# loop-Z/omniisaacgymenvs_loop

Measured on AMD Instinct MI355X. Metric: env-steps/sec USV_CaptureXY at 1/2/4/8 MI355X; wall-clock to reward=30, higher is better.
Workload: dtype fp32; 1 GPU; USV_Virtual_CaptureXY num_envs=131072/GPU PPO-MLP fp32 (BASELINE configs[4] per GPU: 2^20 envs over 8 GPUs); num_envs_per_gpu=131072, horizon_length=16, minibatch_size=8192, mini_epochs=8, parallelism=dp1, exchange=none (one rank), seed=0, full=False

## Files before the change

### omniisaacgymenvs_loop_amd/csrc/usv_field.hip

```cpp
#include "usv_device.h"

USV_PROBE_DEFINE(field)

namespace {

constexpr int G = USV_GRID;
constexpr int G2 = USV_GRID2;
constexpr int FS = USV_FIELD_STRIDE;
constexpr int T = 10;
constexpr int NT = G / T;
constexpr int kWaveThreads = 256;
constexpr int kMaxIters = 4096;
constexpr int kSlotStride = USV_FIELD_SLOT_STATS;
constexpr int kSlotObst = 160;
static_assert(kSlotObst + 2 * USV_NOBST <= kSlotStride, "slot_stats layout");
constexpr int kFieldPackMinEnvs = 32768;
#ifndef USV_SWEEP_WAVES
#define USV_SWEEP_WAVES 2
#endif
constexpr int kPackGrid = 256 * USV_SWEEP_WAVES;

enum {
  SS_GMIN_F = 0, SS_GMAX_F, SS_ANY_INF,
  SS_JMIN_F_NI, SS_JMAX_F_NI, SS_JMAX_F_ALL,
  SS_JRMIN_I_NI, SS_JRMAX_I_NI, SS_JRMAX_I_ALL,
  SS_INSIDE, SS_ITERS, SS_EXACT
};

__device__ __forceinline__ float wall(const uint32_t *freem, int bit) {
  const uint32_t f = (freem[bit >> 5] >> (bit & 31)) & 1u;
  return __uint_as_float((f - 1u) & 0x7f800000u);
}

constexpr int NTP = NT + 2;
constexpr uint32_t kInfBits = 0x7f800000u;
constexpr uint32_t kOcc = 0xFFFFFFFFu;
enum { E_TOP = 0, E_BOT, E_LEFT, E_RIGHT };
constexpr int kOccColWords = (G + 31) / 32;
__device__ __forceinline__ bool occ_bit(const uint32_t *occ, int r, int cc) {
  return (occ[cc * kOccColWords + (r >> 5)] >> (r & 31)) & 1u;
}

constexpr int kRefSweeps = (G * 3) / 2;
template <int NT>
__device__ __forceinline__ void cost_sweeps_exact(const uint32_t *occ, int ix, int iy, float *A, float *B) {
  const int tid = threadIdx.x;
  for (int q = tid; q < G2; q += NT) A[q] = (q == iy * G + ix) ? 0.f : INFINITY;
  __syncthreads();
  for (int it = 0; it < kRefSweeps; ++it) {
    for (int q = tid; q < G2; q += NT) {
      const int r = q / G, cc = q % G;
      float m = A[q];
#pragma unroll
      for (int dy = -1; dy <= 1; ++dy)
#pragma unroll
        for (int dx = -1; dx <= 1; ++dx) {
          if (!dx && !dy) continue;
          const int rr = r - dy, c2 = cc - dx;
          if (rr < 0 || rr >= G || c2 < 0 || c2 >= G) continue;
          m = fminf(m, A[rr * G + c2] + ((dx && dy) ? 1.414f : 1.0f));
        }
      const bool o = r == 0 || r == G - 1 || cc == 0 || cc == G - 1 || occ_bit(occ, r, cc);
      B[q] = o ? INFINITY : m;
    }
    __syncthreads();
    float *t = A; A = B; B = t;
  }
}

constexpr int kPlaceTB = 256;
__global__ __launch_bounds__(kPlaceTB) void k_field_place(usv_cfg_t c, usv_bufs_t b) {
  if (b.ctl[USV_CTL_PLACE] == 0) return;
  const int n = b.n;
  const int count = min(b.ctl[USV_CTL_RESET_COUNT], n);
  const uint64_t h_seed = (uint64_t)(uint32_t)b.ctl[USV_CTL_H_SEED_LO] | ((uint64_t)(uint32_t)b.ctl[USV_CTL_H_SEED_HI] << 32);
  const uint64_t h_step = (uint64_t)(uint32_t)b.ctl[USV_CTL_H_STEP_LO] | ((uint64_t)(uint32_t)b.ctl[USV_CTL_H_STEP_HI] << 32);
  const float *h_inj = reinterpret_cast<const float *>(
      (uintptr_t)((uint64_t)(uint32_t)b.ctl[USV_CTL_H_INJ_LO] | ((uint64_t)(uint32_t)b.ctl[USV_CTL_H_INJ_HI] << 32)));
  const int lane = threadIdx.x & 63;
  const int waves = (int)gridDim.x * (kPlaceTB / 64);
  for (int slot = (int)blockIdx.x * (kPlaceTB / 64) + (int)(threadIdx.x >> 6); slot < count; slot += waves) {
    const int e = b.reset_ids[slot];
    const float2 oc = place_obstacles(c, e, b.px[e], b.py[e], b.field_old_tgt[e], b.field_old_tgt[n + e], h_seed,
                                      h_step, h_inj);
    if (lane < USV_NOBST) {
      b.obst[(size_t)(2 * lane) * n + e] = oc.x;
      b.obst[(size_t)(2 * lane + 1) * n + e] = oc.y;
    }
  }
}

#define USV_SWEEP_NOTE(hb, m) (chg = __builtin_amdgcn_bitop3_b32(chg, (uint32_t)(hb), (uint32_t)(m), 0xF6))
template <bool kPlace, int TH = T, int TW = T, int NTHR = kWaveThreads>
__device__ __forceinline__ void field_wave_body(const usv_cfg_t &c, const usv_bufs_t &b) {
  constexpr int NTR = G / TH, NTC = G / TW;
  constexpr int NPR = NTR + 2, NPC = NTC + 2;
  constexpr int WC = NTHR / 128;
  static_assert(G % TH == 0 && G % TW == 0 && NTR <= 16 && NTC <= 8 * WC && NTHR % 128 == 0, "sweep tiling");
  static_assert(USV_FIELD_TH == TH && USV_FIELD_TW % TW == 0, "sweep tiles inside the field tiles");
  __shared__ uint32_t occ[G * kOccColWords];
  __shared__ float edgeh[2][NPR * NPC][TW];
  __shared__ float edgev[2][NPR * NPC][TH];
  __shared__ int lastc[NPR * NPC];
  __shared__ float so[2 * USV_NOBST];
  __shared__ float slin[G];
  const int n = b.n;
  const int count = min(b.ctl[USV_CTL_RESET_COUNT], n);
  const int tid = threadIdx.x;
  const int lane = tid & 63, wid = tid >> 6;
  const bool place = kPlace && b.ctl[USV_CTL_PLACE] != 0;
  uint64_t h_seed = 0, h_step = 0;
  const float *h_inj = nullptr;
  if (kPlace) {
    h_seed = (uint64_t)(uint32_t)b.ctl[USV_CTL_H_SEED_LO] | ((uint64_t)(uint32_t)b.ctl[USV_CTL_H_SEED_HI] << 32);
    h_step = (uint64_t)(uint32_t)b.ctl[USV_CTL_H_STEP_LO] | ((uint64_t)(uint32_t)b.ctl[USV_CTL_H_STEP_HI] << 32);
    h_inj = reinterpret_cast<const float *>(
        (uintptr_t)((uint64_t)(uint32_t)b.ctl[USV_CTL_H_INJ_LO] | ((uint64_t)(uint32_t)b.ctl[USV_CTL_H_INJ_HI] << 32)));
  }
  const int quad = tid >> 6, qk = tid & 63;
  const int qr = quad / WC, qc = quad % WC;
  const int qw = min(8, NTC - 8 * qc), qh = min(8, NTR - 8 * qr);
  const bool tile_ok = qk < qw * qh;
  const int tr = tile_ok ? qr * 8 + qk / qw : 0;
  const int tc = tile_ok ? qc * 8 + qk % qw : 0;
  const int r0 = tr * TH, c0 = tc * TW;
  const int tp = (tr + 1) * NPC + tc + 1;
  const float cell = (float)((double)c.map_size / G);
  const float half_map = (float)((double)c.map_size / 2);
  const float inv_r = (float)(1.0 / (double)c.influence_radius);
  for (int q = tid; q < 2 * NPR * NPC * TW; q += NTHR) {
    const int t = (q / TW) % (NPR * NPC);
    const int rr = t / NPC, cc = t % NPC;
    if (rr == 0 || rr == NPR - 1 || cc == 0 || cc == NPC - 1) (&edgeh[0][0][0])[q] = INFINITY;
  }
  for (int q = tid; q < 2 * NPR * NPC * TH; q += NTHR) {
    const int t = (q / TH) % (NPR * NPC);
    const int rr = t / NPC, cc = t % NPC;
    if (rr == 0 || rr == NPR - 1 || cc == 0 || cc == NPC - 1) (&edgev[0][0][0])[q] = INFINITY;
  }
  for (int q = tid; q < NPR * NPC; q += NTHR) lastc[q] = -1000;
  for (int slot = blockIdx.x; slot < count; slot += gridDim.x) {
    USV_PHASE(field, 0);
    const int e = b.reset_ids[slot];
    if (kPlace && place) {
      if (wid == 0) {
        const float2 oc = place_obstacles(c, e, b.px[e], b.py[e], b.field_old_tgt[e], b.field_old_tgt[n + e],
                                          h_seed, h_step, h_inj);
        if (lane < USV_NOBST) {
          so[2 * lane] = oc.x;
          so[2 * lane + 1] = oc.y;
          b.obst[(size_t)(2 * lane) * n + e] = oc.x;
          b.obst[(size_t)(2 * lane + 1) * n + e] = oc.y;
        }
      }
    } else if (tid < 2 * USV_NOBST) {
      so[tid] = b.obst[(size_t)tid * n + e];
    }
    if (tid < G) slin[tid] = grid_coord(b.grid_lin, c.map_size, tid);
    for (int q = tid; q < G * kOccColWords; q += NTHR) occ[q] = 0u;
    __syncthreads();
#ifdef USV_PHASE_PROBE
    if (tid == 0 && blockIdx.x < 4096) g_probe_field[blockIdx.x][12] = wall_clock64();
#endif
    if (tid < 2 * USV_NOBST) b.slot_stats[(size_t)slot * kSlotStride + kSlotObst + tid] = so[tid];
    {
      const float half_m = (float)((double)c.map_size / 2);
      const float cellf = (float)((double)c.map_size / G);
      const int reach = (int)ceilf(c.obstacle_radius / cellf) + 2;
      const int bw = 2 * reach + 1;
      for (int q = tid; q < USV_NOBST * bw * bw; q += NTHR) {
        const int o = q / (bw * bw), k = q % (bw * bw);
        const float ox = so[2 * o], oy = so[2 * o + 1];
        const float ic = (ox + half_m) / cellf - 0.5f, jc = (oy + half_m) / cellf - 0.5f;
        if (!(fabsf(ic) < 4.0f * G && fabsf(jc) < 4.0f * G)) continue;
        const int cc = (int)floorf(ic) - reach + k % bw, r = (int)floorf(jc) - reach + k / bw;
        if (cc < 0 || cc >= G || r < 0 || r >= G) continue;
        const float dx = slin[cc] - ox, dy = slin[r] - oy;
        if (sqrtf(fmaf(dy, dy, dx * dx)) - c.obstacle_radius <= 0.f)
          atomicOr(&occ[cc * kOccColWords + (r >> 5)], 1u << (r & 31));
      }
    }
    __syncthreads();
    USV_PHASE(field, 1);
#ifdef USV_PHASE_PROBE
    if (tid == 0 && blockIdx.x < 4096) g_probe_field[blockIdx.x][13] = clock64();
#endif
    const float tx = b.field_old_tgt[e], ty = b.field_old_tgt[n + e];
    int ix = (int)((tx + half_map) / cell), iy = (int)((ty + half_map) / cell);
    ix = min(max(ix, 0), G - 1);
    iy = min(max(iy, 0), G - 1);
    const bool tgt_free = !occ_bit(occ, iy, ix) && ix > 0 && ix < G - 1 && iy > 0 && iy < G - 1;
    float h[TH + 2][TW + 2];
    if (tile_ok) {
#pragma unroll
      for (int i = 0; i < TH; ++i)
#pragma unroll
        for (int j = 0; j < TW; ++j) {
          const int r = r0 + i, cc = c0 + j;
          const bool border = r == 0 || r == G - 1 || cc == 0 || cc == G - 1;
          const bool o = border || occ_bit(occ, r, cc);
          float init = INFINITY;
          if (o) {
            init = __uint_as_float(kOcc);
          } else if (tgt_free) {
            if (r == iy && cc == ix) init = 0.f;
          } else {
            const int di = r - iy, dj = cc - ix;
            if (abs(di) <= 1 && abs(dj) <= 1 && (di || dj)) init = (di && dj) ? 1.414f : 1.0f;
          }
          h[i + 1][j + 1] = init;
        }
#pragma unroll
      for (int k = 0; k < TW; ++k) {
        edgeh[E_TOP][tp][k] = h[1][k + 1];
        edgeh[E_BOT][tp][k] = h[TH][k + 1];
      }
#pragma unroll
      for (int k = 0; k < TH; ++k) {
        edgev[E_LEFT - 2][tp][k] = h[k + 1][1];
        edgev[E_RIGHT - 2][tp][k] = h[k + 1][TW];
      }
      lastc[tp] = 0;
    }
    __syncthreads();
    int it = 0;
    for (; it < kMaxIters; ++it) {
      int changed = 0;
      uint32_t chg = 0u;
      bool dirty = false;
      if (tile_ok) {
#pragma unroll
        for (int dr = -1; dr <= 1; ++dr)
#pragma unroll
          for (int dc = -1; dc <= 1; ++dc) dirty |= lastc[tp + dr * NPC + dc] >= it - 1;
      }
      if (dirty) {
#pragma unroll
        for (int k = 0; k < TW; ++k) {
          h[0][k + 1] = edgeh[E_BOT][tp - NPC][k];
          h[TH + 1][k + 1] = edgeh[E_TOP][tp + NPC][k];
        }
#pragma unroll
        for (int k = 0; k < TH; ++k) {
          h[k + 1][0] = edgev[E_RIGHT - 2][tp - 1][k];
          h[k + 1][TW + 1] = edgev[E_LEFT - 2][tp + 1][k];
        }
        h[0][0] = edgeh[E_BOT][tp - NPC - 1][TW - 1];
        h[0][TW + 1] = edgeh[E_BOT][tp - NPC + 1][0];
        h[TH + 1][0] = edgeh[E_TOP][tp + NPC - 1][TW - 1];
        h[TH + 1][TW + 1] = edgeh[E_TOP][tp + NPC + 1][0];
#pragma unroll
        for (int L = 0; L < 2 * TH + TW - 2; ++L)
#pragma unroll
          for (int i = 1; i <= TH; ++i) {
            const int j = L - 2 * (i - 1) + 1;
            if (j < 1 || j > TW) continue;
            const int32_t hb = __float_as_int(h[i][j]);
            int32_t m = min(hb, __float_as_int(fabsf(h[i - 1][j - 1]) + 1.414f));
            m = min(m, __float_as_int(fabsf(h[i - 1][j]) + 1.0f));
            m = min(m, __float_as_int(fabsf(h[i - 1][j + 1]) + 1.414f));
            m = min(m, __float_as_int(fabsf(h[i][j - 1]) + 1.0f));
            if (i == 1 || i == TH || j == 1 || j == TW) USV_SWEEP_NOTE(hb, m);
            h[i][j] = __int_as_float(m);
          }
#pragma unroll
        for (int L = 0; L < 2 * TH + TW - 2; ++L)
#pragma unroll
          for (int i = TH; i >= 1; --i) {
            const int j = TW - (L - 2 * (TH - i));
            if (j < 1 || j > TW) continue;
            const int32_t hb = __float_as_int(h[i][j]);
            int32_t m = min(hb, __float_as_int(fabsf(h[i + 1][j + 1]) + 1.414f));
            m = min(m, __float_as_int(fabsf(h[i + 1][j]) + 1.0f));
            m = min(m, __float_as_int(fabsf(h[i + 1][j - 1]) + 1.414f));
            m = min(m, __float_as_int(fabsf(h[i][j + 1]) + 1.0f));
            USV_SWEEP_NOTE(hb, m);
            h[i][j] = __int_as_float(m);
          }
        __asm__("" : "+v"(chg));
        changed = chg != 0u;
        if (changed) {
#pragma unroll
          for (int k = 0; k < TW; ++k) {
            edgeh[E_TOP][tp][k] = h[1][k + 1];
            edgeh[E_BOT][tp][k] = h[TH][k + 1];
          }
#pragma unroll
          for (int k = 0; k < TH; ++k) {
            edgev[E_LEFT - 2][tp][k] = h[k + 1][1];
            edgev[E_RIGHT - 2][tp][k] = h[k + 1][TW];
          }
          lastc[tp] = it;
        }
      }
      if (!__syncthreads_or(changed)) break;
    }
    USV_PHASE(field, 2);
#ifdef USV_PHASE_PROBE
    if (tid == 0 && blockIdx.x < 4096) g_probe_field[blockIdx.x][14] = clock64();
#endif
    constexpr float kPinnedCost = 224.0f;
    float hmax = 0.f;
    if (tile_ok) {
#pragma unroll
      for (int i = 0; i < TH; ++i)
#pragma unroll
        for (int j = 0; j < TW; ++j) {
          const uint32_t hb = __float_as_uint(h[i + 1][j + 1]);
          if (hb < kInfBits) hmax = fmaxf(hmax, h[i + 1][j + 1]);
        }
    }
    const bool exact = __syncthreads_or((hmax > kPinnedCost) || (it >= kMaxIters)) != 0;
    constexpr int kSub = USV_FIELD_TW / TW;
    static_assert(USV_FIELD_TCOLS * USV_FIELD_TW == G && USV_FIELD_TCOLS == NTC / kSub, "field tiles = sweep tiles");
    if (tile_ok) {
      float *Ft = b.field + (size_t)e * FS + (tr * USV_FIELD_TCOLS + tc / kSub) * (USV_FIELD_TH * USV_FIELD_TW) +
                  (tc % kSub) * TW;
#pragma unroll
      for (int i = 0; i < TH; ++i)
#pragma unroll
        for (int j = 0; j < TW; ++j)
          Ft[i * USV_FIELD_TW + j] = __float_as_uint(h[i + 1][j + 1]) > kInfBits ? INFINITY : h[i + 1][j + 1];
    }
    if (tile_ok) lastc[tp] = -1000;
    if (exact) {
      __syncthreads();
      float *Fe = b.field + (size_t)e * FS;
      float *scratch = b.sdf + (size_t)e * FS;
      cost_sweeps_exact<NTHR>(occ, ix, iy, Fe, scratch);
      for (int q = tid; q < G2; q += NTHR) Fe[field_idx(q / G, q % G)] = scratch[q];
      if (tid == 0) atomicAdd(&b.ctl[USV_CTL_FIELD_EXACT], 1);
    }
    if (tid == 0) {
      b.slot_stats[(size_t)slot * kSlotStride + SS_ITERS] = (float)it;
      b.slot_stats[(size_t)slot * kSlotStride + SS_EXACT] = exact ? 1.f : 0.f;
#ifdef USV_PHASE_PROBE
      if (blockIdx.x < 4096) g_probe_field[blockIdx.x][15] = (unsigned long long)it;
#endif
    }
    __syncthreads();
    USV_PHASE(field, 3);
  }
}

__global__ __launch_bounds__(kWaveThreads) void k_field_wave(usv_cfg_t c, usv_bufs_t b) { field_wave_body<true>(c, b); }
__global__ __launch_bounds__(kWaveThreads, USV_SWEEP_WAVES) void k_field_wave_pack(usv_cfg_t c, usv_bufs_t b) {
  field_wave_body<false>(c, b);
}
constexpr int kHalfThreads = 512;
__global__ __launch_bounds__(kHalfThreads) void k_field_wave_half(usv_cfg_t c, usv_bufs_t b) {
  field_wave_body<false, T, T / 2, kHalfThreads>(c, b);
}

struct BatchK {
  float inf_val, mask_inf;
};
__device__ __forceinline__ BatchK batch_k(const usv_cfg_t &c, const usv_bufs_t &b) {
  const float max_val = b.ctl[USV_CTL_ANY_FINITE] ? b.fscratch[0] : 100.0f;
  const float inf_val = max_val * 1.5f;
  const float cell = (float)((double)c.map_size / G);
  return BatchK{inf_val, goal_mask(c, inf_val, cell)};
}

#ifndef USV_STATS_WAVES
#define USV_STATS_WAVES 5
#endif
constexpr int kBandRows = 30, kBands = G / kBandRows;
constexpr int kRowGroups = 3;
constexpr int kWavePairs = 19;
constexpr int kBandIters = kBandRows / kRowGroups;
static_assert(G % kBandRows == 0 && kBandRows % kRowGroups == 0 && kWavePairs * kRowGroups <= 64 &&
              4 * 2 * kWavePairs >= G && G % 2 == 0, "k_field_stats geometry");
static_assert(kSlotObst >= 16 + 12 * kBands, "slot_stats band partials");
__global__ __launch_bounds__(256, USV_STATS_WAVES) void k_field_stats(usv_cfg_t c, usv_bufs_t b) {
  __shared__ float red[10][4];
  __shared__ int flags[2];
  __shared__ float slin[G];
  __shared__ float so[2 * USV_NOBST];
  const int count = min(b.ctl[USV_CTL_RESET_COUNT], b.n);
  const int tid = threadIdx.x, lane = tid & 63, wid = tid >> 6;
  const int cbase = wid * 2 * kWavePairs;
  const int cpl = lane % kWavePairs, rg = lane / kWavePairs;
  const int c0u = cbase + 2 * cpl;
  const bool act = rg < kRowGroups && c0u < G;
  const int c0 = act ? c0u : 0;
  const int rgc = act ? rg : 0;
  const int chi = min(cbase + 2 * kWavePairs - 1, G - 1);
  const float cell = (float)((double)c.map_size / G);
  const float inv_r = (float)(1.0 / (double)c.influence_radius);
  const float inv_safe = 1.0f / c.safe_radius;
  const float far_d = c.influence_radius + 2.0f * c.obstacle_radius + 0.01f * cell + 1e-3f;
  const uint32_t far2 = __float_as_uint(far_d * far_d);
  const int items = count * kBands;
  if (tid < G) slin[tid] = grid_coord(b.grid_lin, c.map_size, tid);
  const auto load_costs = [&](int wq, int eq, float2 *dst) {
    const float *F = b.field + (size_t)eq * FS;
#pragma unroll
    for (int k = 0; k < kBandIters; ++k) {
      const int r = (wq % kBands) * kBandRows + rgc + kRowGroups * k;
      dst[k] = *reinterpret_cast<const float2 *>(F + field_idx(r, c0));
    }
  };
  float2 gA[kBandIters];
  const auto item = [&](const int w, float2 (&gv)[kBandIters]) {
    const int slot = w / kBands, band = w % kBands;
    if (tid < 2 * USV_NOBST) so[tid] = b.slot_stats[(size_t)slot * kSlotStride + kSlotObst + tid];
    if (tid < 2) flags[tid] = 0;
    __syncthreads();
    load_costs(w, b.reset_ids[slot], gv);
    const float gxa = slin[c0], gxb = slin[c0 + 1];
    uint32_t omask;
    {
      const float ylo = slin[band * kBandRows], yhi = slin[band * kBandRows + kBandRows - 1];
      const float xlo = slin[cbase], xhi = slin[chi];
      const int ol = lane & (USV_NOBST - 1);
      const float oxl = so[2 * ol], oyl = so[2 * ol + 1];
      const float dyb = fmaxf(fmaxf(ylo - oyl, oyl - yhi), 0.f);
      const float dxb_ = fmaxf(fmaxf(xlo - oxl, oxl - xhi), 0.f);
      omask = (uint32_t)(__ballot(lane < USV_NOBST && !(dyb > far_d) && !(dxb_ > far_d)) & 0xFFFFull);
      omask = __builtin_amdgcn_readfirstlane(omask);
    }
    float gmin = INFINITY, gmax = -INFINITY, jmin_f = INFINITY, jmax_f = -INFINITY, jall_f = 0.f;
    float jrmin_i = INFINITY, jrmax_i = -INFINITY, jrall_i = 0.f;
    int any_inf = 0, inside = 0;
    const auto stat = [&](float g, float sv) {
      const float dte = sv - c.obstacle_radius;
      const bool ins = dte <= 0.f;
      inside |= ins;
      const float jr = j_raw(c, dte, inv_r);
      const bool gi = isinf(g);
      any_inf |= gi;
      const float j = jr * clampt(div_rn(g * cell, c.safe_radius, inv_safe), 0.f, 1.f);
      jrall_i = fmaxf(jrall_i, gi ? jr : 0.f);
      jrmin_i = fminf(jrmin_i, (gi && !ins) ? jr : INFINITY);
      jrmax_i = fmaxf(jrmax_i, (gi && !ins) ? jr : -INFINITY);
      gmin = fminf(gmin, gi ? INFINITY : g);
      gmax = fmaxf(gmax, gi ? -INFINITY : g);
      jall_f = fmaxf(jall_f, gi ? 0.f : j);
      jmin_f = fminf(jmin_f, (!gi && !ins) ? j : INFINITY);
      jmax_f = fmaxf(jmax_f, (!gi && !ins) ? j : -INFINITY);
    };
    const auto stat_far = [&](float g) {
      const bool gi = isinf(g);
      any_inf |= gi;
      jrmin_i = fminf(jrmin_i, gi ? 0.f : INFINITY);
      jrmax_i = fmaxf(jrmax_i, gi ? 0.f : -INFINITY);
      gmin = fminf(gmin, gi ? INFINITY : g);
      gmax = fmaxf(gmax, gi ? -INFINITY : g);
      jmin_f = fminf(jmin_f, gi ? INFINITY : 0.f);
      jmax_f = fmaxf(jmax_f, gi ? -INFINITY : 0.f);
    };
    float gy[kBandIters];
    uint32_t a[kBandIters], bb[kBandIters];
#pragma unroll
    for (int k = 0; k < kBandIters; ++k) {
      gy[k] = slin[band * kBandRows + rgc + kRowGroups * k];
      a[k] = bb[k] = 0x7F800000u;
    }
    for (uint32_t om = omask; om != 0u; om &= om - 1u) {
      const int o = __builtin_ctz(om);
      const float ox = so[2 * o], oyo = so[2 * o + 1];
      const float da = gxa - ox, db = gxb - ox;
      const float dxa = da * da, dxb = db * db;
#pragma unroll
      for (int k = 0; k < kBandIters; ++k) {
        const float dy = gy[k] - oyo;
        a[k] = min(a[k], __float_as_uint(fmaf(dy, dy, dxa)));
        bb[k] = min(bb[k], __float_as_uint(fmaf(dy, dy, dxb)));
      }
    }
#pragma unroll
    for (int k = 0; k < kBandIters; ++k) {
      const bool near = act && (a[k] < far2 || bb[k] < far2);
      if (__ballot(near) != 0ull) {
        const float sva = sqrtf(__uint_as_float(a[k])) - c.obstacle_radius;
        const float svb = sqrtf(__uint_as_float(bb[k])) - c.obstacle_radius;
        if (act) {
          stat(gv[k].x, sva);
          stat(gv[k].y, svb);
        }
      } else if (act) {
        stat_far(gv[k].x);
        stat_far(gv[k].y);
      }
    }
    float vals[9] = {wave_min(gmin), wave_max(gmax), wave_min(jmin_f), wave_max(jmax_f), wave_max(jall_f),
                     wave_min(jrmin_i), wave_max(jrmax_i), wave_max(jrall_i), 0.f};
    __syncthreads();
    if (lane == 0)
      for (int k = 0; k < 8; ++k) red[k][wid] = vals[k];
    if (any_inf) flags[0] = 1;
    if (inside) flags[1] = 1;
    __syncthreads();
    if (tid == 0) {
      float a[8];
      for (int k = 0; k < 8; ++k) a[k] = red[k][0];
      for (int v = 1; v < 4; ++v) {
        a[0] = fminf(a[0], red[0][v]); a[1] = fmaxf(a[1], red[1][v]);
        a[2] = fminf(a[2], red[2][v]); a[3] = fmaxf(a[3], red[3][v]); a[4] = fmaxf(a[4], red[4][v]);
        a[5] = fminf(a[5], red[5][v]); a[6] = fmaxf(a[6], red[6][v]); a[7] = fmaxf(a[7], red[7][v]);
      }
      float *pp = b.slot_stats + (size_t)slot * kSlotStride + 16 + 12 * band;
      pp[SS_GMIN_F] = a[0]; pp[SS_GMAX_F] = a[1]; pp[SS_ANY_INF] = flags[0] ? 1.f : 0.f;
      pp[SS_JMIN_F_NI] = a[2]; pp[SS_JMAX_F_NI] = a[3]; pp[SS_JMAX_F_ALL] = a[4];
      pp[SS_JRMIN_I_NI] = a[5]; pp[SS_JRMAX_I_NI] = a[6]; pp[SS_JRMAX_I_ALL] = a[7];
      pp[SS_INSIDE] = flags[1] ? 1.f : 0.f;
    }
    __syncthreads();
  };
  for (int w = blockIdx.x; w < items; w += gridDim.x) item(w, gA);
}

#ifndef USV_BATCH_BLOCKS
#define USV_BATCH_BLOCKS 64
#endif
#ifndef USV_BATCH_SLOTS_PER_WAVE
#define USV_BATCH_SLOTS_PER_WAVE 6
#endif
constexpr int kBatchBlocks = USV_BATCH_BLOCKS;
constexpr int kBatchSpw = USV_BATCH_SLOTS_PER_WAVE;
static_assert(kBatchSpw >= 1 && 10 * kBatchSpw <= 64, "k_field_batch lane groups");
__global__ __launch_bounds__(256) void k_field_batch(usv_cfg_t c, usv_bufs_t b) {
  __shared__ float wred[4][4];
  __shared__ bool last;
  const int count = min(b.ctl[USV_CTL_RESET_COUNT], b.n);
  if (count <= 0) return;
  const int tid = threadIdx.x, lane = tid & 63, wid = tid >> 6;
  const int grp = lane / 10, q = lane % 10, l0 = 10 * grp;
  const int nw = (int)gridDim.x * 4;
  float gfin = -INFINITY, jf = 0.f, jr = 0.f, ins = 0.f;
  const bool is_min = q == SS_GMIN_F || q == SS_JMIN_F_NI || q == SS_JRMIN_I_NI;
  for (int sl0 = ((int)blockIdx.x * 4 + wid) * kBatchSpw; sl0 < count; sl0 += nw * kBatchSpw) {
    const int sl = sl0 + grp;
    const bool ok = grp < kBatchSpw && sl < count;
    float a = 0.f;
    if (ok) {
      float *st = b.slot_stats + (size_t)sl * kSlotStride;
      float x[kBands];
#pragma unroll
      for (int ch = 0; ch < kBands; ++ch) x[ch] = st[16 + 12 * ch + q];
      a = x[0];
#pragma unroll
      for (int ch = 1; ch < kBands; ++ch) a = is_min ? fminf(a, x[ch]) : fmaxf(a, x[ch]);
      st[q] = a;
    }
    const float s_gmax = __shfl(a, ok ? l0 + SS_GMAX_F : lane, 64);
    const float s_anyinf = __shfl(a, ok ? l0 + SS_ANY_INF : lane, 64);
    const float s_jf = __shfl(a, ok ? l0 + SS_JMAX_F_ALL : lane, 64);
    const float s_jr = __shfl(a, ok ? l0 + SS_JRMAX_I_ALL : lane, 64);
    const float s_in = __shfl(a, ok ? l0 + SS_INSIDE : lane, 64);
    if (ok) {
      gfin = fmaxf(gfin, s_gmax);
      jf = fmaxf(jf, s_jf);
      if (s_anyinf != 0.f) jr = fmaxf(jr, s_jr);
      ins = fmaxf(ins, s_in);
    }
  }
#pragma unroll
  for (int off = 32; off >= 1; off >>= 1) {
    gfin = fmaxf(gfin, __shfl_xor(gfin, off, 64));
    jf = fmaxf(jf, __shfl_xor(jf, off, 64));
    jr = fmaxf(jr, __shfl_xor(jr, off, 64));
    ins = fmaxf(ins, __shfl_xor(ins, off, 64));
  }
  if (lane == 0) { wred[wid][0] = gfin; wred[wid][1] = jf; wred[wid][2] = jr; wred[wid][3] = ins; }
  __syncthreads();
  if (tid == 0) {
    float g = wred[0][0], f = wred[0][1], r = wred[0][2], in = wred[0][3];
    for (int w = 1; w < 4; ++w) {
      g = fmaxf(g, wred[w][0]); f = fmaxf(f, wred[w][1]); r = fmaxf(r, wred[w][2]); in = fmaxf(in, wred[w][3]);
    }
    if (isfinite(g)) {
      atomic_max_f32(&b.fscratch[0], g);
      atomicOr(&b.ctl[USV_CTL_ANY_FINITE], 1);
    }
    atomic_max_f32(&b.fscratch[2], f);
    atomic_max_f32(&b.fscratch[3], r);
    if (in != 0.f) atomicOr(&b.ctl[USV_CTL_ANY_INSIDE], 1);
    __threadfence();
    last = atomicAdd(&b.ctl[USV_CTL_BATCH_DONE], 1) == (int)gridDim.x - 1;
  }
  __syncthreads();
  if (!last || tid != 0) return;
  __threadfence();
  const BatchK k = batch_k(c, b);
  b.fscratch[1] = fmaxf(b.fscratch[2], b.fscratch[3] * k.mask_inf);
  b.ctl[USV_CTL_BATCH_DONE] = 0;
}

__global__ __launch_bounds__(256) void k_field_norm(usv_cfg_t c, usv_bufs_t b) {
  const int count = min(b.ctl[USV_CTL_RESET_COUNT], b.n);
  const BatchK k = batch_k(c, b);
  const bool any_inside = b.ctl[USV_CTL_ANY_INSIDE] != 0;
  const float cur_max = b.fscratch[1];
  const float high = (cur_max > 1e-6f) ? cur_max * 10.0f : 100.0f;
  for (int slot = (int)(blockIdx.x * blockDim.x + threadIdx.x); slot < count; slot += (int)(gridDim.x * blockDim.x)) {
    const int e = b.reset_ids[slot];
    const float *st = b.slot_stats + (size_t)slot * kSlotStride;
    const bool has_inf = st[SS_ANY_INF] != 0.f;
    const bool has_inside = st[SS_INSIDE] != 0.f;
    const float gmin = has_inf ? fminf(st[SS_GMIN_F], k.inf_val) : st[SS_GMIN_F];
    const float gmax = has_inf ? fmaxf(st[SS_GMAX_F], k.inf_val) : st[SS_GMAX_F];
    float jmn = st[SS_JMIN_F_NI], jmx = st[SS_JMAX_F_NI];
    if (isfinite(st[SS_JRMIN_I_NI])) {
      jmn = fminf(jmn, st[SS_JRMIN_I_NI] * k.mask_inf);
      jmx = fmaxf(jmx, st[SS_JRMAX_I_NI] * k.mask_inf);
    }
    if (any_inside && has_inside) { jmn = fminf(jmn, high); jmx = fmaxf(jmx, high); }
    float4 *fn = reinterpret_cast<float4 *>(b.fnorm + (size_t)e * USV_FNORM);
    const float gden = (gmax - gmin) + 1e-6f, jden = (jmx - jmn) + 1e-6f;
    fn[0] = make_float4(gmin, gden, jmn, jden);
    fn[1] = make_float4(k.inf_val, any_inside ? high : -high, 1.0f / gden, 1.0f / jden);
  }
}

__global__ __launch_bounds__(256) void k_field_view(usv_cfg_t c, usv_bufs_t b, const int32_t *ids, int count,
                                                    float *out) {
  const float cell = (float)((double)c.map_size / G);
  const float inv_r = (float)(1.0 / (double)c.influence_radius);
  const float inv_safe = 1.0f / c.safe_radius;
  const long long total = (long long)count * G2;
  for (long long q = (long long)blockIdx.x * blockDim.x + threadIdx.x; q < total; q += (long long)gridDim.x * blockDim.x) {
    const int i = (int)(q / G2), cell_i = (int)(q % G2), r = cell_i / G, cc = cell_i % G;
    const int e = ids[i];
    const float4 *fn = reinterpret_cast<const float4 *>(b.fnorm + (size_t)e * USV_FNORM);
    const FieldNorm k = field_norm_of(fn[0], fn[1]);
    const float *ob = b.obst + e;
    const float sv = cell_sdf([&](int o) { return make_float2(ob[(size_t)(2 * o) * b.n], ob[(size_t)(2 * o + 1) * b.n]); },
                              grid_coord(b.grid_lin, c.map_size, cc), grid_coord(b.grid_lin, c.map_size, r),
                              c.obstacle_radius);
    out[q] = field_value(c, k, sv, b.field[(size_t)e * FS + field_idx(r, cc)], cell, inv_r, inv_safe);
  }
}

}

namespace {
constexpr int kStatsGridCap = 4096;
static int stats_grid(int n) { return n * kBands < kStatsGridCap ? n * kBands : kStatsGridCap; }

int field_stages(const usv_cfg_t *cfg, const usv_bufs_t *b, int stage, hipStream_t s) {
  const int grid_b = b->n < 512 ? b->n : 512;
  const int grid_n = (b->n + 255) / 256 < 64 ? (b->n + 255) / 256 : 64;
  const int grid_p = (b->n + kPlaceTB / 64 - 1) / (kPlaceTB / 64) < 1024 ? (b->n + kPlaceTB / 64 - 1) / (kPlaceTB / 64) : 1024;
  if (stage == 1) {
    hipLaunchKernelGGL(k_field_place, dim3(grid_p), dim3(kPlaceTB), 0, s, *cfg, *b);
    USV_CHECK_LAUNCH();
    return 0;
  }
  if (stage == 2 || stage == 3) {
    const char *half_env = getenv("USV_FIELD_HALF");
    const bool half = half_env ? atoi(half_env) != 0 : b->n < kFieldPackMinEnvs;
    if (half) {
      hipLaunchKernelGGL(k_field_wave_half, dim3(b->n < 256 ? b->n : 256), dim3(kHalfThreads), 0, s, *cfg, *b);
    } else {
      const int grid_w = b->n < kPackGrid ? b->n : kPackGrid;
      hipLaunchKernelGGL(k_field_wave_pack, dim3(grid_w), dim3(kWaveThreads), 0, s, *cfg, *b);
    }
    USV_CHECK_LAUNCH();
    const int grid_s = stats_grid(b->n);
    hipLaunchKernelGGL(k_field_stats, dim3(grid_s), dim3(256), 0, s, *cfg, *b);
    USV_CHECK_LAUNCH();
  }
  if (stage == 2 || stage == 4) {
    hipLaunchKernelGGL(k_field_batch, dim3(kBatchBlocks), dim3(256), 0, s, *cfg, *b);
    USV_CHECK_LAUNCH();
    hipLaunchKernelGGL(k_field_norm, dim3(grid_n), dim3(256), 0, s, *cfg, *b);
    USV_CHECK_LAUNCH();
  }
  return 0;
}
}

extern "C" int usv_field_stage(const usv_cfg_t *cfg, const usv_bufs_t *b, int stage, void *stream) {
  if (!cfg || !b || b->n <= 0 || !b->slot_stats || !b->field || !b->sdf || !b->fnorm || stage < 1 || stage > 4) return 1;
  return field_stages(cfg, b, stage, (hipStream_t)stream);
}

extern "C" int usv_field_view(const usv_cfg_t *cfg, const usv_bufs_t *b, const int32_t *env_ids, int count,
                              float *out, void *stream) {
  if (!cfg || !b || b->n <= 0 || !b->field || !b->sdf || !b->fnorm || !env_ids || !out || count < 0) return 1;
  if (count == 0) return 0;
  const long long total = (long long)count * G2;
  const int grid = (int)((total + 255) / 256 < 8192 ? (total + 255) / 256 : 8192);
  hipLaunchKernelGGL(k_field_view, dim3(grid), dim3(256), 0, (hipStream_t)stream, *cfg, *b, env_ids, count, out);
  USV_CHECK_LAUNCH();
  return 0;
}

extern "C" int usv_potential_field(const usv_cfg_t *cfg, const usv_bufs_t *b, void *stream) {
  if (!cfg || !b || b->n <= 0 || !b->slot_stats || !b->field || !b->sdf || !b->fnorm) return 1;
  hipStream_t s = (hipStream_t)stream;
  const int grid_b = b->n < 512 ? b->n : 512;
  const int grid_n = (b->n + 255) / 256 < 64 ? (b->n + 255) / 256 : 64;
  const char *pack_env = getenv("USV_FIELD_PACK");
  const bool pack = pack_env ? atoi(pack_env) != 0 : b->n >= kFieldPackMinEnvs;
  if (pack) {
    const int grid_p = (b->n + kPlaceTB / 64 - 1) / (kPlaceTB / 64) < 1024 ? (b->n + kPlaceTB / 64 - 1) / (kPlaceTB / 64) : 1024;
    hipLaunchKernelGGL(k_field_place, dim3(grid_p), dim3(kPlaceTB), 0, s, *cfg, *b);
    USV_CHECK_LAUNCH();
  }
  if (pack) hipLaunchKernelGGL(k_field_wave_pack, dim3(b->n < kPackGrid ? b->n : kPackGrid), dim3(kWaveThreads), 0, s,
                              *cfg, *b);
  else hipLaunchKernelGGL(k_field_wave, dim3(grid_b), dim3(kWaveThreads), 0, s, *cfg, *b);
  USV_CHECK_LAUNCH();
  const int grid_s = stats_grid(b->n);
  hipLaunchKernelGGL(k_field_stats, dim3(grid_s), dim3(256), 0, s, *cfg, *b);
  USV_CHECK_LAUNCH();
  hipLaunchKernelGGL(k_field_batch, dim3(kBatchBlocks), dim3(256), 0, s, *cfg, *b);
  USV_CHECK_LAUNCH();
  hipLaunchKernelGGL(k_field_norm, dim3(grid_n), dim3(256), 0, s, *cfg, *b);
  USV_CHECK_LAUNCH();
  return 0;
}
```

Measured before the change: 35.71 million env-steps/s.

## Compute far-tile field stats in sweep kernel; stats kernel visits only near tiles

The sweep kernel now decides which field tiles lie beyond obstacle influence. For those far tiles it reduces min/max/inf stats directly from registers into a separate slot_stats record, and it writes a bitmask of near tiles. The stats kernel is reworked from fixed row bands to a compacted list of near tiles only, with a depth-4 load pipeline, so it no longer rereads the full field from memory. A ring ordering of tiles around the target is also added, changing which thread owns each tile. This adds atomics, extra reductions and another syncthreads per slot to the sweep kernel.

Measured after the change: 36.05 million env-steps/s, median of 6. About the same (+0.9%).

```diff
diff --git a/omniisaacgymenvs_loop_amd/csrc/usv_field.hip b/omniisaacgymenvs_loop_amd/csrc/usv_field.hip
--- a/omniisaacgymenvs_loop_amd/csrc/usv_field.hip
+++ b/omniisaacgymenvs_loop_amd/csrc/usv_field.hip
@@ -13,12 +13,19 @@
 constexpr int kMaxIters = 4096;
 constexpr int kSlotStride = USV_FIELD_SLOT_STATS;
 constexpr int kSlotObst = 160;
-static_assert(kSlotObst + 2 * USV_NOBST <= kSlotStride, "slot_stats layout");
+constexpr int kSlotFar = 16 + 12 * 5;
+constexpr int kSlotNear = kSlotFar + 12;
+constexpr int kNearWords = 8;
+static_assert(kSlotObst + 2 * USV_NOBST <= kSlotStride && kSlotNear + kNearWords <= kSlotObst &&
+              USV_FIELD_TROWS * USV_FIELD_TCOLS <= 32 * kNearWords, "slot_stats layout");
 constexpr int kFieldPackMinEnvs = 32768;
 #ifndef USV_SWEEP_WAVES
 #define USV_SWEEP_WAVES 2
 #endif
 constexpr int kPackGrid = 256 * USV_SWEEP_WAVES;
+#ifndef USV_SWEEP_RING
+#define USV_SWEEP_RING 1
+#endif
 
 enum {
   SS_GMIN_F = 0, SS_GMAX_F, SS_ANY_INF,
@@ -30,6 +37,15 @@
 __device__ __forceinline__ float wall(const uint32_t *freem, int bit) {
   const uint32_t f = (freem[bit >> 5] >> (bit & 31)) & 1u;
   return __uint_as_float((f - 1u) & 0x7f800000u);
+}
+
+__device__ __forceinline__ float field_far_d(const usv_cfg_t &c, float cell) {
+  return c.influence_radius + 2.0f * c.obstacle_radius + 0.01f * cell + 1e-3f;
+}
+__device__ __forceinline__ bool box_beyond(float xlo, float xhi, float ylo, float yhi, float ox, float oy, float far_d) {
+  const float dyb = fmaxf(fmaxf(ylo - oy, oy - yhi), 0.f);
+  const float dxb = fmaxf(fmaxf(xlo - ox, ox - xhi), 0.f);
+  return dyb > far_d || dxb > far_d;
 }
 
 constexpr int NTP = NT + 2;
@@ -92,7 +108,7 @@
 
 #define USV_SWEEP_NOTE(hb, m) (chg = __builtin_amdgcn_bitop3_b32(chg, (uint32_t)(hb), (uint32_t)(m), 0xF6))
 template <bool kPlace, int TH = T, int TW = T, int NTHR = kWaveThreads>
-__device__ __forceinline__ void field_wave_body(const usv_cfg_t &c, const usv_bufs_t &b) {
+__device__ __forceinline__ void field_wave_body(const usv_cfg_t &c, const usv_bufs_t &b, const int far_on) {
   constexpr int NTR = G / TH, NTC = G / TW;
   constexpr int NPR = NTR + 2, NPC = NTC + 2;
   constexpr int WC = NTHR / 128;
@@ -104,6 +120,8 @@
   __shared__ int lastc[NPR * NPC];
   __shared__ float so[2 * USV_NOBST];
   __shared__ float slin[G];
+  __shared__ uint32_t nearm[kNearWords];
+  __shared__ float farw[NTHR / 64][3];
   const int n = b.n;
   const int count = min(b.ctl[USV_CTL_RESET_COUNT], n);
   const int tid = threadIdx.x;
@@ -117,6 +135,9 @@
     h_inj = reinterpret_cast<const float *>(
         (uintptr_t)((uint64_t)(uint32_t)b.ctl[USV_CTL_H_INJ_LO] | ((uint64_t)(uint32_t)b.ctl[USV_CTL_H_INJ_HI] << 32)));
   }
+#if USV_SWEEP_RING
+  __shared__ uint16_t perm[NTHR];
+#else
   const int quad = tid >> 6, qk = tid & 63;
   const int qr = quad / WC, qc = quad % WC;
   const int qw = min(8, NTC - 8 * qc), qh = min(8, NTR - 8 * qr);
@@ -125,6 +146,7 @@
   const int tc = tile_ok ? qc * 8 + qk % qw : 0;
   const int r0 = tr * TH, c0 = tc * TW;
   const int tp = (tr + 1) * NPC + tc + 1;
+#endif
   const float cell = (float)((double)c.map_size / G);
   const float half_map = (float)((double)c.map_size / 2);
   const float inv_r = (float)(1.0 / (double)c.influence_radius);
@@ -158,7 +180,35 @@
     }
     if (tid < G) slin[tid] = grid_coord(b.grid_lin, c.map_size, tid);
     for (int q = tid; q < G * kOccColWords; q += NTHR) occ[q] = 0u;
-    __syncthreads();
+    if (tid < kNearWords) nearm[tid] = 0u;
+    const float tx = b.field_old_tgt[e], ty = b.field_old_tgt[n + e];
+    int ix = (int)((tx + half_map) / cell), iy = (int)((ty + half_map) / cell);
+    ix = min(max(ix, 0), G - 1);
+    iy = min(max(iy, 0), G - 1);
+#if USV_SWEEP_RING
+    if (tid < NTR * NTC) {
+      const int a = iy / TH, bq = ix / TW, pr = tid / NTC, pc = tid % NTC;
+      const int d = max(abs(pr - a), abs(pc - bq));
+      int rank = 0;
+      if (d > 0) {
+        rank = (min(a + d - 1, NTR - 1) - max(a - d + 1, 0) + 1) * (min(bq + d - 1, NTC - 1) - max(bq - d + 1, 0) + 1);
+        const int cl = bq - d, ch = bq + d, clc = max(cl, 0), chc = min(ch, NTC - 1);
+        const int sides = (cl >= 0) + (ch <= NTC - 1);
+        if (a - d >= 0 && pr > a - d) rank += chc - clc + 1;
+        rank += max(0, min(pr - 1, a + d - 1) - max(a - d + 1, 0) + 1) * sides;
+        rank += abs(pr - a) == d ? pc - clc : (pc == ch && cl >= 0 ? 1 : 0);
+      }
+      perm[rank] = (uint16_t)tid;
+    }
+#endif
+    __syncthreads();
+#if USV_SWEEP_RING
+    const bool tile_ok = tid < NTR * NTC;
+    const int mytile = tile_ok ? (int)perm[tid] : 0;
+    const int tr = mytile / NTC, tc = mytile % NTC;
+    const int r0 = tr * TH, c0 = tc * TW;
+    const int tp = (tr + 1) * NPC + tc + 1;
+#endif
 #ifdef USV_PHASE_PROBE
     if (tid == 0 && blockIdx.x < 4096) g_probe_field[blockIdx.x][12] = wall_clock64();
 #endif
@@ -185,10 +235,6 @@
 #ifdef USV_PHASE_PROBE
     if (tid == 0 && blockIdx.x < 4096) g_probe_field[blockIdx.x][13] = clock64();
 #endif
-    const float tx = b.field_old_tgt[e], ty = b.field_old_tgt[n + e];
-    int ix = (int)((tx + half_map) / cell), iy = (int)((ty + half_map) / cell);
-    ix = min(max(ix, 0), G - 1);
-    iy = min(max(iy, 0), G - 1);
     const bool tgt_free = !occ_bit(occ, iy, ix) && ix > 0 && ix < G - 1 && iy > 0 && iy < G - 1;
     float h[TH + 2][TW + 2];
     if (tile_ok) {
@@ -301,6 +347,7 @@
 #endif
     constexpr float kPinnedCost = 224.0f;
     float hmax = 0.f;
+    uint32_t hminb = kOcc, hmaxb = 0u;
     if (tile_ok) {
 #pragma unroll
       for (int i = 0; i < TH; ++i)
@@ -308,10 +355,32 @@
         for (int j = 0; j < TW; ++j) {
           const uint32_t hb = __float_as_uint(h[i + 1][j + 1]);
           if (hb < kInfBits) hmax = fmaxf(hmax, h[i + 1][j + 1]);
+          hminb = min(hminb, hb);
+          hmaxb = max(hmaxb, hb);
         }
     }
     const bool exact = __syncthreads_or((hmax > kPinnedCost) || (it >= kMaxIters)) != 0;
     constexpr int kSub = USV_FIELD_TW / TW;
+    {
+      bool tfar = tile_ok && far_on != 0 && !exact;
+      if (tfar) {
+        const float far_d = field_far_d(c, cell);
+        const int fc0 = (tc / kSub) * USV_FIELD_TW;
+        const float xlo = slin[fc0], xhi = slin[fc0 + USV_FIELD_TW - 1], ylo = slin[r0], yhi = slin[r0 + TH - 1];
+        for (int o = 0; o < USV_NOBST; ++o) tfar &= box_beyond(xlo, xhi, ylo, yhi, so[2 * o], so[2 * o + 1], far_d);
+      }
+      if (tile_ok && !tfar) atomicOr(&nearm[(tr * USV_FIELD_TCOLS + tc / kSub) >> 5],
+                                     1u << ((tr * USV_FIELD_TCOLS + tc / kSub) & 31));
+      const bool fin = tfar && hminb < kInfBits;
+      const float fmin = wave_min(fin ? __uint_as_float(hminb) : INFINITY);
+      const float fmax = wave_max(fin ? hmax : -INFINITY);
+      const bool finf = __ballot(tfar && hmaxb >= kInfBits) != 0ull;
+      if (lane == 0) {
+        farw[wid][0] = fmin;
+        farw[wid][1] = fmax;
+        farw[wid][2] = finf ? 1.f : 0.f;
+      }
+    }
     static_assert(USV_FIELD_TCOLS * USV_FIELD_TW == G && USV_FIELD_TCOLS == NTC / kSub, "field tiles = sweep tiles");
     if (tile_ok) {
       float *Ft = b.field + (size_t)e * FS + (tr * USV_FIELD_TCOLS + tc / kSub) * (USV_FIELD_TH * USV_FIELD_TW) +
@@ -331,7 +400,22 @@
       for (int q = tid; q < G2; q += NTHR) Fe[field_idx(q / G, q % G)] = scratch[q];
       if (tid == 0) atomicAdd(&b.ctl[USV_CTL_FIELD_EXACT], 1);
     }
+    __syncthreads();
+    if (tid < kNearWords)
+      reinterpret_cast<uint32_t *>(b.slot_stats)[(size_t)slot * kSlotStride + kSlotNear + tid] = nearm[tid];
     if (tid == 0) {
+      float fmin = farw[0][0], fmax = farw[0][1], finf = farw[0][2];
+      for (int w = 1; w < NTHR / 64; ++w) {
+        fmin = fminf(fmin, farw[w][0]);
+        fmax = fmaxf(fmax, farw[w][1]);
+        finf = fmaxf(finf, farw[w][2]);
+      }
+      const bool fin = fmax >= 0.f;
+      float *fr = b.slot_stats + (size_t)slot * kSlotStride + kSlotFar;
+      fr[SS_GMIN_F] = fmin; fr[SS_GMAX_F] = fmax; fr[SS_ANY_INF] = finf;
+      fr[SS_JMIN_F_NI] = fin ? 0.f : INFINITY; fr[SS_JMAX_F_NI] = fin ? 0.f : -INFINITY; fr[SS_JMAX_F_ALL] = 0.f;
+      fr[SS_JRMIN_I_NI] = finf != 0.f ? 0.f : INFINITY; fr[SS_JRMAX_I_NI] = finf != 0.f ? 0.f : -INFINITY;
+      fr[SS_JRMAX_I_ALL] = 0.f; fr[SS_INSIDE] = 0.f;
       b.slot_stats[(size_t)slot * kSlotStride + SS_ITERS] = (float)it;
       b.slot_stats[(size_t)slot * kSlotStride + SS_EXACT] = exact ? 1.f : 0.f;
 #ifdef USV_PHASE_PROBE
@@ -343,13 +427,15 @@
   }
 }
 
-__global__ __launch_bounds__(kWaveThreads) void k_field_wave(usv_cfg_t c, usv_bufs_t b) { field_wave_body<true>(c, b); }
-__global__ __launch_bounds__(kWaveThreads, USV_SWEEP_WAVES) void k_field_wave_pack(usv_cfg_t c, usv_bufs_t b) {
-  field_wave_body<false>(c, b);
+__global__ __launch_bounds__(kWaveThreads) void k_field_wave(usv_cfg_t c, usv_bufs_t b, int far_on) {
+  field_wave_body<true>(c, b, far_on);
+}
+__global__ __launch_bounds__(kWaveThreads, USV_SWEEP_WAVES) void k_field_wave_pack(usv_cfg_t c, usv_bufs_t b, int far_on) {
+  field_wave_body<false>(c, b, far_on);
 }
 constexpr int kHalfThreads = 512;
-__global__ __launch_bounds__(kHalfThreads) void k_field_wave_half(usv_cfg_t c, usv_bufs_t b) {
-  field_wave_body<false, T, T / 2, kHalfThreads>(c, b);
+__global__ __launch_bounds__(kHalfThreads) void k_field_wave_half(usv_cfg_t c, usv_bufs_t b, int far_on) {
+  field_wave_body<false, T, T / 2, kHalfThreads>(c, b, far_on);
 }
 
 struct BatchK {
@@ -365,61 +451,54 @@
 #ifndef USV_STATS_WAVES
 #define USV_STATS_WAVES 5
 #endif
-constexpr int kBandRows = 30, kBands = G / kBandRows;
-constexpr int kRowGroups = 3;
-constexpr int kWavePairs = 19;
-constexpr int kBandIters = kBandRows / kRowGroups;
-static_assert(G % kBandRows == 0 && kBandRows % kRowGroups == 0 && kWavePairs * kRowGroups <= 64 &&
-              4 * 2 * kWavePairs >= G && G % 2 == 0, "k_field_stats geometry");
-static_assert(kSlotObst >= 16 + 12 * kBands, "slot_stats band partials");
+#ifndef USV_STATS_CHUNKS
+#define USV_STATS_CHUNKS 1
+#endif
+constexpr int kChunks = USV_STATS_CHUNKS;
+constexpr int kTiles = USV_FIELD_TROWS * USV_FIELD_TCOLS;
+constexpr int kTileCells = USV_FIELD_TH * USV_FIELD_TW;
+constexpr int kTilePairs = USV_FIELD_TW / 2;
+constexpr int kStatsDepth = 4;
+static_assert(kChunks >= 1 && 16 + 12 * kChunks <= kSlotFar, "slot_stats chunk partials");
+static_assert(USV_FIELD_TW % 2 == 0 && USV_FIELD_TH * kTilePairs <= 64 && kTiles <= 256 &&
+              USV_FIELD_TROWS * USV_FIELD_TH == G && USV_FIELD_TCOLS * USV_FIELD_TW == G, "k_field_stats geometry");
 __global__ __launch_bounds__(256, USV_STATS_WAVES) void k_field_stats(usv_cfg_t c, usv_bufs_t b) {
   __shared__ float red[10][4];
-  __shared__ int flags[2];
   __shared__ float slin[G];
   __shared__ float so[2 * USV_NOBST];
+  __shared__ uint32_t nm[kNearWords];
+  __shared__ uint8_t list[256];
   const int count = min(b.ctl[USV_CTL_RESET_COUNT], b.n);
-  const int tid = threadIdx.x, lane = tid & 63, wid = tid >> 6;
-  const int cbase = wid * 2 * kWavePairs;
-  const int cpl = lane % kWavePairs, rg = lane / kWavePairs;
-  const int c0u = cbase + 2 * cpl;
-  const bool act = rg < kRowGroups && c0u < G;
-  const int c0 = act ? c0u : 0;
-  const int rgc = act ? rg : 0;
-  const int chi = min(cbase + 2 * kWavePairs - 1, G - 1);
+  const int tid = threadIdx.x, lane = tid & 63;
+  const int wid = __builtin_amdgcn_readfirstlane(tid >> 6);
+  const bool act = lane < USV_FIELD_TH * kTilePairs;
+  const int ti = act ? lane / kTilePairs : 0;
+  const int tj = act ? 2 * (lane % kTilePairs) : 0;
   const float cell = (float)((double)c.map_size / G);
   const float inv_r = (float)(1.0 / (double)c.influence_radius);
   const float inv_safe = 1.0f / c.safe_radius;
-  const float far_d = c.influence_radius + 2.0f * c.obstacle_radius + 0.01f * cell + 1e-3f;
+  const float far_d = field_far_d(c, cell);
   const uint32_t far2 = __float_as_uint(far_d * far_d);
-  const int items = count * kBands;
+  const int items = count * kChunks;
   if (tid < G) slin[tid] = grid_coord(b.grid_lin, c.map_size, tid);
-  const auto load_costs = [&](int wq, int eq, float2 *dst) {
-    const float *F = b.field + (size_t)eq * FS;
-#pragma unroll
-    for (int k = 0; k < kBandIters; ++k) {
-      const int r = (wq % kBands) * kBandRows + rgc + kRowGroups * k;
-      dst[k] = *reinterpret_cast<const float2 *>(F + field_idx(r, c0));
-    }
-  };
-  float2 gA[kBandIters];
-  const auto item = [&](const int w, float2 (&gv)[kBandIters]) {
-    const int slot = w / kBands, band = w % kBands;
+  for (int w = blockIdx.x; w < items; w += gridDim.x) {
+    const int slot = w / kChunks, chunk = w % kChunks;
     if (tid < 2 * USV_NOBST) so[tid] = b.slot_stats[(size_t)slot * kSlotStride + kSlotObst + tid];
-    if (tid < 2) flags[tid] = 0;
-    __syncthreads();
-    load_costs(w, b.reset_ids[slot], gv);
-    const float gxa = slin[c0], gxb = slin[c0 + 1];
-    uint32_t omask;
-    {
-      const float ylo = slin[band * kBandRows], yhi = slin[band * kBandRows + kBandRows - 1];
-      const float xlo = slin[cbase], xhi = slin[chi];
-      const int ol = lane & (USV_NOBST - 1);
-      const float oxl = so[2 * ol], oyl = so[2 * ol + 1];
-      const float dyb = fmaxf(fmaxf(ylo - oyl, oyl - yhi), 0.f);
-      const float dxb_ = fmaxf(fmaxf(xlo - oxl, oxl - xhi), 0.f);
-      omask = (uint32_t)(__ballot(lane < USV_NOBST && !(dyb > far_d) && !(dxb_ > far_d)) & 0xFFFFull);
-      omask = __builtin_amdgcn_readfirstlane(omask);
-    }
+    if (tid < kNearWords)
+      nm[tid] = reinterpret_cast<const uint32_t *>(b.slot_stats)[(size_t)slot * kSlotStride + kSlotNear + tid] &
+                (32 * tid + 32 <= kTiles ? 0xFFFFFFFFu : (1u << (kTiles - 32 * (kNearWords - 1))) - 1u);
+    __syncthreads();
+    int nnear = 0;
+#pragma unroll
+    for (int k = 0; k < kNearWords; ++k) nnear += __popc(nm[k]);
+    if (tid < kTiles && ((nm[tid >> 5] >> (tid & 31)) & 1u)) {
+      int rank = __popc(nm[tid >> 5] & ((1u << (tid & 31)) - 1u));
+      for (int k = 0; k < (tid >> 5); ++k) rank += __popc(nm[k]);
+      list[rank] = (uint8_t)tid;
+    }
+    __syncthreads();
+    nnear = __builtin_amdgcn_readfirstlane(nnear);
+    const float *F = b.field + (size_t)b.reset_ids[slot] * FS;
     float gmin = INFINITY, gmax = -INFINITY, jmin_f = INFINITY, jmax_f = -INFINITY, jall_f = 0.f;
     float jrmin_i = INFINITY, jrmax_i = -INFINITY, jrall_i = 0.f;
     int any_inf = 0, inside = 0;
@@ -450,66 +529,81 @@
       jmin_f = fminf(jmin_f, gi ? INFINITY : 0.f);
       jmax_f = fmaxf(jmax_f, gi ? -INFINITY : 0.f);
     };
-    float gy[kBandIters];
-    uint32_t a[kBandIters], bb[kBandIters];
-#pragma unroll
-    for (int k = 0; k < kBandIters; ++k) {
-      gy[k] = slin[band * kBandRows + rgc + kRowGroups * k];
-      a[k] = bb[k] = 0x7F800000u;
-    }
-    for (uint32_t om = omask; om != 0u; om &= om - 1u) {
-      const int o = __builtin_ctz(om);
-      const float ox = so[2 * o], oyo = so[2 * o + 1];
-      const float da = gxa - ox, db = gxb - ox;
-      const float dxa = da * da, dxb = db * db;
-#pragma unroll
-      for (int k = 0; k < kBandIters; ++k) {
-        const float dy = gy[k] - oyo;
-        a[k] = min(a[k], __float_as_uint(fmaf(dy, dy, dxa)));
-        bb[k] = min(bb[k], __float_as_uint(fmaf(dy, dy, dxb)));
-      }
-    }
-#pragma unroll
-    for (int k = 0; k < kBandIters; ++k) {
-      const bool near = act && (a[k] < far2 || bb[k] < far2);
+    const auto tile_stats = [&](const int tile, const float2 gv) {
+      const int r0 = (tile / USV_FIELD_TCOLS) * USV_FIELD_TH, c0 = (tile % USV_FIELD_TCOLS) * USV_FIELD_TW;
+      const int ol = lane & (USV_NOBST - 1);
+      uint32_t omask = (uint32_t)(__ballot(lane < USV_NOBST &&
+                                           !box_beyond(slin[c0], slin[c0 + USV_FIELD_TW - 1], slin[r0],
+                                                       slin[r0 + USV_FIELD_TH - 1], so[2 * ol], so[2 * ol + 1], far_d)) &
+                                  0xFFFFull);
+      omask = __builtin_amdgcn_readfirstlane(omask);
+      const float gxa = slin[c0 + tj], gxb = slin[c0 + tj + 1], gy = slin[r0 + ti];
+      uint32_t a = 0x7F800000u, bb = 0x7F800000u;
+      for (uint32_t om = omask; om != 0u; om &= om - 1u) {
+        const int o = __builtin_ctz(om);
+        const float ox = so[2 * o], oyo = so[2 * o + 1];
+        const float da = gxa - ox, db = gxb - ox;
+        const float dxa = da * da, dxb = db * db;
+        const float dy = gy - oyo;
+        a = min(a, __float_as_uint(fmaf(dy, dy, dxa)));
+        bb = min(bb, __float_as_uint(fmaf(dy, dy, dxb)));
+      }
+      const bool near = act && (a < far2 || bb < far2);
       if (__ballot(near) != 0ull) {
-        const float sva = sqrtf(__uint_as_float(a[k])) - c.obstacle_radius;
-        const float svb = sqrtf(__uint_as_float(bb[k])) - c.obstacle_radius;
+        const float sva = sqrtf(__uint_as_float(a)) - c.obstacle_radius;
+        const float svb = sqrtf(__uint_as_float(bb)) - c.obstacle_radius;
         if (act) {
-          stat(gv[k].x, sva);
-          stat(gv[k].y, svb);
+          stat(gv.x, sva);
+          stat(gv.y, svb);
         }
       } else if (act) {
-        stat_far(gv[k].x);
-        stat_far(gv[k].y);
-      }
-    }
-    float vals[9] = {wave_min(gmin), wave_max(gmax), wave_min(jmin_f), wave_max(jmax_f), wave_max(jall_f),
-                     wave_min(jrmin_i), wave_max(jrmax_i), wave_max(jrall_i), 0.f};
-    __syncthreads();
-    if (lane == 0)
+        stat_far(gv.x);
+        stat_far(gv.y);
+      }
+    };
+    constexpr int kStep = 4 * kChunks;
+    for (int j0 = chunk * 4 + wid; j0 < nnear; j0 += kStatsDepth * kStep) {
+      int tl[kStatsDepth];
+      float2 gv[kStatsDepth];
+#pragma unroll
+      for (int u = 0; u < kStatsDepth; ++u) {
+        const int j = j0 + u * kStep;
+        tl[u] = j < nnear ? __builtin_amdgcn_readfirstlane((int)list[j]) : -1;
+        gv[u] = tl[u] >= 0 ? *reinterpret_cast<const float2 *>(F + tl[u] * kTileCells + ti * USV_FIELD_TW + tj)
+                           : make_float2(0.f, 0.f);
+      }
+#pragma unroll
+      for (int u = 0; u < kStatsDepth; ++u)
+        if (tl[u] >= 0) tile_stats(tl[u], gv[u]);
+    }
+    const float vals[8] = {wave_min(gmin), wave_max(gmax), wave_min(jmin_f), wave_max(jmax_f), wave_max(jall_f),
+                           wave_min(jrmin_i), wave_max(jrmax_i), wave_max(jrall_i)};
+    const bool w_inf = __ballot(any_inf != 0) != 0ull, w_ins = __ballot(inside != 0) != 0ull;
+    if (lane == 0) {
       for (int k = 0; k < 8; ++k) red[k][wid] = vals[k];
-    if (any_inf) flags[0] = 1;
-    if (inside) flags[1] = 1;
+      red[8][wid] = w_inf ? 1.f : 0.f;
+      red[9][wid] = w_ins ? 1.f : 0.f;
+    }
     __syncthreads();
     if (tid == 0) {
-      float a[8];
-      for (int k = 0; k < 8; ++k) a[k] = red[k][0];
+      float a[10];
+      for (int k = 0; k < 10; ++k) a[k] = red[k][0];
       for (int v = 1; v < 4; ++v) {
         a[0] = fminf(a[0], red[0][v]); a[1] = fmaxf(a[1], red[1][v]);
         a[2] = fminf(a[2], red[2][v]); a[3] = fmaxf(a[3], red[3][v]); a[4] = fmaxf(a[4], red[4][v]);
         a[5] = fminf(a[5], red[5][v]); a[6] = fmaxf(a[6], red[6][v]); a[7] = fmaxf(a[7], red[7][v]);
-      }
-      float *pp = b.slot_stats + (size_t)slot * kSlotStride + 16 + 12 * band;
-      pp[SS_GMIN_F] = a[0]; pp[SS_GMAX_F] = a[1]; pp[SS_ANY_INF] = flags[0] ? 1.f : 0.f;
+        a[8] = fmaxf(a[8], red[8][v]); a[9] = fmaxf(a[9], red[9][v]);
+      }
+      float *pp = b.slot_stats + (size_t)slot * kSlotStride + 16 + 12 * chunk;
+      pp[SS_GMIN_F] = a[0]; pp[SS_GMAX_F] = a[1]; pp[SS_ANY_INF] = a[8];
       pp[SS_JMIN_F_NI] = a[2]; pp[SS_JMAX_F_NI] = a[3]; pp[SS_JMAX_F_ALL] = a[4];
       pp[SS_JRMIN_I_NI] = a[5]; pp[SS_JRMAX_I_NI] = a[6]; pp[SS_JRMAX_I_ALL] = a[7];
-      pp[SS_INSIDE] = flags[1] ? 1.f : 0.f;
-    }
-    __syncthreads();
-  };
-  for (int w = blockIdx.x; w < items; w += gridDim.x) item(w, gA);
-}
+      pp[SS_INSIDE] = a[9];
+    }
+    __syncthreads();
+  }
+}
+
 
 #ifndef USV_BATCH_BLOCKS
 #define USV_BATCH_BLOCKS 64
@@ -536,12 +630,13 @@
     float a = 0.f;
     if (ok) {
       float *st = b.slot_stats + (size_t)sl * kSlotStride;
-      float x[kBands];
-#pragma unroll
-      for (int ch = 0; ch < kBands; ++ch) x[ch] = st[16 + 12 * ch + q];
+      float x[kChunks + 1];
+#pragma unroll
+      for (int ch = 0; ch < kChunks; ++ch) x[ch] = st[16 + 12 * ch + q];
+      x[kChunks] = st[kSlotFar + q];
       a = x[0];
 #pragma unroll
-      for (int ch = 1; ch < kBands; ++ch) a = is_min ? fminf(a, x[ch]) : fmaxf(a, x[ch]);
+      for (int ch = 1; ch <= kChunks; ++ch) a = is_min ? fminf(a, x[ch]) : fmaxf(a, x[ch]);
       st[q] = a;
     }
     const float s_gmax = __shfl(a, ok ? l0 + SS_GMAX_F : lane, 64);
@@ -637,7 +732,11 @@
 
 namespace {
 constexpr int kStatsGridCap = 4096;
-static int stats_grid(int n) { return n * kBands < kStatsGridCap ? n * kBands : kStatsGridCap; }
+static int stats_grid(int n) { return n * kChunks < kStatsGridCap ? n * kChunks : kStatsGridCap; }
+static int field_far_on() {
+  const char *e = getenv("USV_FIELD_FAR");
+  return e ? atoi(e) != 0 : 1;
+}
 
 int field_stages(const usv_cfg_t *cfg, const usv_bufs_t *b, int stage, hipStream_t s) {
   const int grid_b = b->n < 512 ? b->n : 512;
@@ -649,13 +748,14 @@
     return 0;
   }
   if (stage == 2 || stage == 3) {
+    const int far_on = field_far_on();
     const char *half_env = getenv("USV_FIELD_HALF");
     const bool half = half_env ? atoi(half_env) != 0 : b->n < kFieldPackMinEnvs;
     if (half) {
-      hipLaunchKernelGGL(k_field_wave_half, dim3(b->n < 256 ? b->n : 256), dim3(kHalfThreads), 0, s, *cfg, *b);
+      hipLaunchKernelGGL(k_field_wave_half, dim3(b->n < 256 ? b->n : 256), dim3(kHalfThreads), 0, s, *cfg, *b, far_on);
     } else {
       const int grid_w = b->n < kPackGrid ? b->n : kPackGrid;
-      hipLaunchKernelGGL(k_field_wave_pack, dim3(grid_w), dim3(kWaveThreads), 0, s, *cfg, *b);
+      hipLaunchKernelGGL(k_field_wave_pack, dim3(grid_w), dim3(kWaveThreads), 0, s, *cfg, *b, far_on);
     }
     USV_CHECK_LAUNCH();
     const int grid_s = stats_grid(b->n);
@@ -693,6 +793,7 @@
   hipStream_t s = (hipStream_t)stream;
   const int grid_b = b->n < 512 ? b->n : 512;
   const int grid_n = (b->n + 255) / 256 < 64 ? (b->n + 255) / 256 : 64;
+  const int far_on = field_far_on();
   const char *pack_env = getenv("USV_FIELD_PACK");
   const bool pack = pack_env ? atoi(pack_env) != 0 : b->n >= kFieldPackMinEnvs;
   if (pack) {
@@ -701,8 +802,8 @@
     USV_CHECK_LAUNCH();
   }
   if (pack) hipLaunchKernelGGL(k_field_wave_pack, dim3(b->n < kPackGrid ? b->n : kPackGrid), dim3(kWaveThreads), 0, s,
-                              *cfg, *b);
-  else hipLaunchKernelGGL(k_field_wave, dim3(grid_b), dim3(kWaveThreads), 0, s, *cfg, *b);
+                              *cfg, *b, far_on);
+  else hipLaunchKernelGGL(k_field_wave, dim3(grid_b), dim3(kWaveThreads), 0, s, *cfg, *b, far_on);
   USV_CHECK_LAUNCH();
   const int grid_s = stats_grid(b->n);
   hipLaunchKernelGGL(k_field_stats, dim3(grid_s), dim3(256), 0, s, *cfg, *b);
```
